# heathsc/bs_call

Measured on AMD Instinct MI355X. Metric: genome positions called/sec, higher is better.
Workload: dtype f64

## Files before the change

### bs_call_amd/csrc/bscall_api.c

```c
#ifndef __HIP_PLATFORM_AMD__
#define __HIP_PLATFORM_AMD__ 1
#endif
#include <hip/hip_runtime_api.h>
#include <math.h>
#include <pthread.h>
#include <stdarg.h>
#include <stdio.h>
#include <stdlib.h>
#include <string.h>

#include "../../include/bscall_amd.h"
#include "devtables.h"
#include "bsmath.h"
#include "bsmath_tables.h"
#include "synth.h"
#include "dbsnpdev_core.h"

int bsc_dev_launch_call(const void *cts, const void *ref, uint64_t n, void *out, uint32_t out_dw, void *skip,
                        const void *tb, void *het_list, void *counters, int num_cus, void *stream, void *ev_start,
                        void *ev_mid, void *ev_stop);
int bsc_dev_launch_accumulate(const void *rd, const void *bin_off, const void *seq, uint32_t x, uint32_t y, uint32_t min_qual, void *cts,
                              void *counters, int num_cus, void *stream);
int bsc_dev_launch_bin_reads(const void *tpl, uint32_t nr, const void *seq, uint64_t seq_bytes, uint32_t x, uint32_t y, void *tflag,
                             void *bin_cnt, void *bin_off, void *bin_cur, void *scan_tmp, size_t scan_tmp_bytes, void *rd,
// ... 25 lines not shown
size_t bsc_dev_chain_het_bytes(uint32_t n, int num_cus, int with_depth, int reads);
size_t bsc_dev_chain_scratch_bytes(int num_cus);
size_t bsc_dev_chain_multi_table_bytes(uint32_t n_blocks);
int bsc_dev_launch_chain_multi(const bsc_chain_launch *L, const bsc_chain_mblock *blk, uint32_t b_first, uint32_t b_last, void *tab_h,
                               void *tab_d, size_t *cursor);
int bsc_dev_launch_accumulate_summary(const void *rd, const void *bin_off, const void *seq, uint32_t x, uint32_t y, uint32_t min_qual, void *cts,
                                      void *counters, int num_cus, void *stream);
size_t bsc_dev_summary_bytes(void);
int bsc_dev_launch_accumulate_multi(const void *rd, const void *bin_off, const void *seq, const void *d_blk, uint32_t n_blk, uint32_t n_bins,
                                    uint32_t min_qual, void *cts, void *counters, int num_cus, void *stream);
int bsc_dev_scan_tmp_bytes_u64(uint32_t n, size_t *bytes);
size_t bsc_dev_prep_plan_bytes(void);
int bsc_dev_launch_prep(const void *raw, uint32_t nr, const void *seq, uint64_t seq_bytes, const void *misms, uint64_t n_misms,
                        const bsc_prep_params *par, void *ms_work, void *plan, void *out_len, void *out_off, void *scan_tmp,
                        size_t scan_tmp_bytes, void *tpl_out, void *seq_out, uint64_t seq_out_cap, void *cnt, int num_cus, void *stream,
                        const void *prof_ref, uint32_t prof_x, uint32_t prof_n_ref, uint32_t prof_cap, uint32_t prof_used0, void *prof_table,
                        void *max_pos1, void *used_scan, void *prof_mask);
int bsc_dev_launch_bcf(const void *recs, const void *core, const void *aux, const void *n_recs, uint64_t max_recs, int32_t rid,
                       const bsc_bcf_ids *ids, const void *name_pos, const void *name_off, const void *name_bytes, uint32_t n_names,
                       void *tile_bytes, void *tile_off, void *scan_tmp, size_t scan_tmp_bytes, void *out, uint64_t out_cap, void *totals,
                       int num_cus, void *stream, const void *emit_len);
int bsc_dev_launch_vcf_text(const void *recs, const void *core, const void *aux, const void *n_recs, uint64_t max_recs, const char *contig,
                            uint32_t contig_len, const void *name_pos, const void *name_off, const void *name_bytes, uint32_t n_names,
                            void *tile_bytes, void *tile_off, void *line_len, void *scan_tmp, size_t scan_tmp_bytes, void *out, uint64_t out_cap,
                            void *totals, int num_cus, void *stream);
int bsc_dev_launch_fmt_g(const void *v, uint64_t n, void *out16, int num_cus, void *stream);
int bsc_dev_launch_meth(const void *recs, const void *core, const void *aux, const void *n_recs, uint64_t max_recs, const void *emit, const char *contig,
                        uint32_t contig_len, const bsc_meth_params *par, void *tile_bytes, void *tile_off, void *line_len, void *scan_tmp,
                        size_t scan_tmp_bytes, void *out, uint64_t out_cap, void *totals, int num_cus, void *stream);
int bsc_dev_launch_ref_pad(const void *packed, const void *d_blk, uint32_t n_blk, void *padded, uint32_t n_pos, int num_cus, void *stream);
int bsc_dev_launch_bin_reads_multi(const void *tpl, uint32_t nr, const void *seq, uint64_t seq_bytes, const void *d_blk, uint32_t n_blk,
                                   uint32_t n_bins, void *tflag, void *bin_cnt, void *bin_off, void *bin_cur, void *scan_tmp,
// ... 131 lines not shown
  size_t cap_pmask;
  void *d_pprof, *d_pmax, *d_pused;
  size_t cap_pprof, cap_pmax, cap_pused;
  void *d_refp;
  size_t cap_refp;
  const uint32_t *mb_toff;
  int dbg_fail_summary;
  int reads_fused;
  void *d_fscr;
  size_t cap_fscr;
  hipEvent_t ev_rchain[2];
  int ev_rchain_valid;
  hipEvent_t ev_raw[2];
  int ev_raw_valid;
  int ref_resident;
  hipEvent_t ev_acc[2];
  int ev_acc_valid;
  hipStream_t s_in, s_out;
  hipEvent_t ev_in[2], ev_k[2], ev_out[2];
  void *p_cts[2], *p_ref[2], *p_out[2], *p_skip[2];
  size_t p_cap_cts[2], p_cap_ref[2], p_cap_out[2], p_cap_skip[2];
  int pipe_ready;
  int profiling;
#define BSC_EV_RING 32
  hipEvent_t ev[BSC_EV_RING][3];
  uint64_t ev_count;
};

static __thread char bsc_errbuf[512];

// ... 153 lines not shown
  HIP_TRY(hipGetDeviceProperties(&prop, dev));
  if (strncmp(prop.gcnArchName, "gfx950", 6) != 0)
    return bsc_fail(BSC_ERR_NO_DEVICE, "bsc_create: device %d is %s; the kernels are built for gfx950 only", dev,
                    prop.gcnArchName);

  bsc_context *ctx = calloc(1, sizeof *ctx);
  if (!ctx) return bsc_fail(BSC_ERR_NOMEM, "bsc_create: out of host memory");
  ctx->params = p;
  ctx->device = dev;
  ctx->num_cus = prop.multiProcessorCount;
  ctx->max_launch = BSC_MAX_LAUNCH;
  ctx->rec_share = 0.55;
  ctx->stage_timing = getenv("BSC_STAGE_TIMING") != NULL;
  ctx->no_emit_bytes = getenv("BSC_NO_EMIT_BYTES") != NULL;
  ctx->no_h2d_turns = getenv("BSC_NO_H2D_TURNS") != NULL;
  {
    const char *ml = getenv("BSC_MAX_LAUNCH_SITES");
    if (ml && *ml) {
      const unsigned long long v = strtoull(ml, NULL, 10) & ~63ull;
      if (v >= 64 && v < BSC_MAX_LAUNCH) ctx->max_launch = v;
    }
  }
  bsc_build_tables(ctx);
  int rc = BSC_OK;
  if (bsc_build_phred_table(&ctx->host_tables)) {
    rc = bsc_fail(BSC_ERR_ARG, "bsc_create: the QUAL staircase of this build's log is not monotone");
    bsc_destroy(ctx);
    return rc;
  }
  if (hipStreamCreateWithFlags(&ctx->stream, hipStreamNonBlocking) != hipSuccess ||
// ... 50 lines not shown
  hipFree(ctx->d_bcnt);
  hipFree(ctx->d_boff);
  hipFree(ctx->d_bcur);
  hipFree(ctx->d_bscan);
  for (int b = 0; b < 2; b++) {
    hipFree(ctx->p_cts[b]);
    hipFree(ctx->p_ref[b]);
    hipFree(ctx->p_out[b]);
    hipFree(ctx->p_skip[b]);
    if (ctx->ev_in[b]) hipEventDestroy(ctx->ev_in[b]);
    if (ctx->ev_k[b]) hipEventDestroy(ctx->ev_k[b]);
    if (ctx->ev_out[b]) hipEventDestroy(ctx->ev_out[b]);
  }
  if (ctx->s_in) hipStreamDestroy(ctx->s_in);
  if (ctx->s_out) hipStreamDestroy(ctx->s_out);
  hipFree(ctx->d_vg);
  hipFree(ctx->d_sstats);
    hipFree(ctx->d_pairs);
  hipFree(ctx->d_tcnt);
  hipFree(ctx->d_toff);
  hipFree(ctx->d_scantmp);
  hipFree(ctx->d_recs);
  hipFree(ctx->d_btb);
  hipFree(ctx->d_bto);
  hipFree(ctx->d_bscn);
  hipFree(ctx->d_bnm);
  hipFree(ctx->dbs.d_blob);
  bsc_dev_dbsnp_flat_free(&ctx->dbs.blob);
  if (ctx->h_names) hipHostFree(ctx->h_names);
  for (int k = 0; k < 4; k++)
// ... 121 lines not shown
                                ctx->profiling ? ctx->ev[ctx->ev_count % BSC_EV_RING][0] : NULL,
                                ctx->profiling ? ctx->ev[ctx->ev_count % BSC_EV_RING][1] : NULL,
                                ctx->profiling ? ctx->ev[ctx->ev_count % BSC_EV_RING][2] : NULL);
    if (ctx->profiling) ctx->ev_count++;
    if (e) return bsc_fail(BSC_ERR_HIP, "kernel launch failed: %s", hipGetErrorString((hipError_t)e));
    done += m;
  }
  ctx->sites += n;
  return BSC_OK;
}

#define BSC_PIPE_CHUNK (1u << 20)

static int bsc_pipe_init(bsc_context *ctx) {
  if (ctx->pipe_ready) return BSC_OK;
  HIP_TRY(hipStreamCreateWithFlags(&ctx->s_in, hipStreamNonBlocking));
  HIP_TRY(hipStreamCreateWithFlags(&ctx->s_out, hipStreamNonBlocking));
  for (int b = 0; b < 2; b++) {
    HIP_TRY(hipEventCreateWithFlags(&ctx->ev_in[b], hipEventDisableTiming));
    HIP_TRY(hipEventCreateWithFlags(&ctx->ev_k[b], hipEventDisableTiming));
    HIP_TRY(hipEventCreateWithFlags(&ctx->ev_out[b], hipEventDisableTiming));
  }
  ctx->pipe_ready = 1;
  return BSC_OK;
}

int bsc_call_sites(bsc_context *ctx, const bsc_pileup *cts, const uint8_t *ref, uint64_t n, void *out,
                   uint32_t out_stride, uint8_t *skip) {
  if (!ctx) return bsc_fail(BSC_ERR_ARG, "bsc_call_sites: ctx is NULL");
  int rc = bsc_check_stride(out_stride);
  if (rc) return rc;
// ... 688 lines not shown
  L.cts = d_cts;
  if (ctx->profiling) {
    if (!ctx->ev_chain[0])
      for (int i = 0; i < 2; i++) HIP_TRY(hipEventCreate(&ctx->ev_chain[i]));
    L.ev_start = ctx->ev_chain[0];
    L.ev_stop = ctx->ev_chain[1];
    ctx->ev_chain_valid = 1;
  }
  int e = bsc_dev_launch_chain(&L);
  if (e) return bsc_fail(BSC_ERR_HIP, "chain launch failed: %s", hipGetErrorString((hipError_t)e));
  if (with_stats) ctx->carry_slot ^= 1u;
  ctx->sites += w->n;
  return BSC_OK;
}

static int bsc_reads_chain_queue(bsc_context *ctx, const void *d_tpl, uint32_t nr, const void *d_seq, uint64_t seq_bytes, uint32_t x,
                                 uint32_t y, const void *d_ref, const void *d_dbsnp, const bsc_vcf_params *params, int with_stats,
                                 void *d_core, void *d_aux, void *d_emit, hipStream_t s) {
  const uint64_t sz64 = (uint64_t)y - x + 1;
  bsc_window w = {x, (uint32_t)sz64, 0u, (uint32_t)sz64};
  int rc = bsc_window_check("reads chain", &w);
  if (rc) return rc;
  size_t scan_bytes = 0;
  if ((rc = bsc_accumulate_reserve(ctx, nr, x, y, &scan_bytes))) return rc;
  if ((rc = bsc_reserve(&ctx->d_fscr, &ctx->cap_fscr, bsc_dev_chain_scratch_bytes(ctx->num_cus)))) return rc;
  bsc_chain_launch L;
  if ((rc = bsc_chain_fill(ctx, &L, &w, params, with_stats, 1, d_ref, d_dbsnp, d_core, d_aux, s))) return rc;
  L.emit_out = d_emit;
  if (ctx->profiling) {
    if (!ctx->ev_rchain[0])
// ... 6 lines not shown
  if (two_kernels) {
    const size_t n_pad = ((size_t)w.n + 63u) / 64u * 64u;
    size_t need = n_pad * bsc_dev_summary_bytes();
    if (ctx->dbg_fail_summary) {
      void *never = NULL;
      size_t cap0 = 0;
      if (!bsc_try_reserve(&never, &cap0, (size_t)1 << 60)) need = 0;
      else hipFree(never);
    }
    if (!need || !bsc_try_reserve(&ctx->d_cts, &ctx->cap_cts, need)) two_kernels = 0;
  }
  if (two_kernels) {
    e = bsc_dev_launch_accumulate_summary(ctx->d_rd, ctx->d_boff, d_seq, x, y, (uint32_t)ctx->params.min_qual, ctx->d_cts,
                                          ctx->d_counters, ctx->num_cus, s);
    if (e) return bsc_fail(BSC_ERR_HIP, "accumulate launch failed: %s", hipGetErrorString((hipError_t)e));
    bsc_chain_launch L2 = L;
    L.cts = ctx->d_cts;
    L.cts_summary = 1;
    L.run_if = 2;
    e = bsc_dev_launch_chain(&L);
    if (e) return bsc_fail(BSC_ERR_HIP, "reads chain launch failed: %s", hipGetErrorString((hipError_t)e));
    L = L2;
    L.run_if = 1;
    L.ev_start = NULL;
  }
  if (!two_kernels || L.run_if) {
    L.rd = ctx->d_rd;
    L.bin_off = ctx->d_boff;
    L.seq = d_seq;
    L.f_scratch = ctx->d_fscr;
    L.n_bins = bsc_dev_n_bins(w.n);
    L.min_qual = (uint32_t)ctx->params.min_qual;
  }
  e = bsc_dev_launch_chain(&L);
  if (e) return bsc_fail(BSC_ERR_HIP, "reads chain launch failed: %s", hipGetErrorString((hipError_t)e));
  if (ctx->profiling) {
    HIP_TRY(hipEventRecord(ctx->ev_rchain[1], s));
    ctx->ev_rchain_valid = 1;
  }
  if (with_stats) ctx->carry_slot ^= 1u;
  ctx->sites += w.n;
  return BSC_OK;
}

int bsc_reads_chain_device(bsc_context *ctx, const void *d_tpl, uint32_t nr, const void *d_seq, uint64_t seq_bytes, uint32_t x,
                           uint32_t y, const void *d_ref, const void *d_dbsnp, const bsc_vcf_params *params, int with_stats,
                           void *d_core, void *d_aux, void *stream) {
  if (!ctx || !params || !d_ref || !d_core) return bsc_fail(BSC_ERR_ARG, "bsc_reads_chain_device: NULL argument");
// ... 107 lines not shown
  free(so);
  if (rc >= 0 || strstr(bsc_errbuf, "seq_out too small"))
    return bsc_fail(BSC_ERR_ARG, "bsc_prepare_templates_device: template %u fails check %u on the device, none on the host", ti, code);
  char msg[sizeof bsc_errbuf];
  snprintf(msg, sizeof msg, "%s", bsc_errbuf);
  char *at = strstr(msg, "template 0 ");
  if (at) {
    char tail[sizeof bsc_errbuf];
    snprintf(tail, sizeof tail, "%s", at + 11);
    *at = 0;
    return bsc_fail(rc, "%stemplate %u %s", msg, ti, tail);
  }
  return bsc_fail(rc, "%s (template %u)", msg, ti);
}

static int bsc_prep_queue(bsc_context *ctx, const void *d_raw, uint32_t nr, const void *d_seq, uint64_t seq_bytes, const void *d_misms, uint64_t n_misms,
                          const bsc_prep_params *par, void *d_tpl_out, void *d_seq_out, uint64_t seq_out_cap, const bsc_read_profile *pf, hipStream_t s) {
  int rc;
  size_t scan_bytes = 0;
  const uint32_t n2 = 2u * nr + 1u;
  if (bsc_dev_scan_tmp_bytes_u64(n2, &scan_bytes)) return bsc_fail(BSC_ERR_HIP, "bsc_prepare_templates_device: scan size query failed");
  if ((rc = bsc_reserve(&ctx->d_pplan, &ctx->cap_pplan, (size_t)(nr ? nr : 1) * 2u * bsc_dev_prep_plan_bytes()))) return rc;
  if ((rc = bsc_reserve(&ctx->d_plen, &ctx->cap_plen, (size_t)n2 * 8u))) return rc;
  if ((rc = bsc_reserve(&ctx->d_poff, &ctx->cap_poff, (size_t)n2 * 8u))) return rc;
  if ((rc = bsc_reserve(&ctx->d_pms, &ctx->cap_pms, (size_t)(n_misms ? n_misms : 1) * sizeof(bsc_misms)))) return rc;
  if ((rc = bsc_reserve(&ctx->d_pscan, &ctx->cap_pscan, scan_bytes ? scan_bytes : 1))) return rc;
  if ((rc = bsc_reserve(&ctx->d_pcnt, &ctx->cap_pcnt, BSC_PREP_CNT_ALL * sizeof(unsigned long long)))) return rc;
  const size_t prof_bytes = pf && nr ? (size_t)pf->cap * 4u * sizeof(unsigned long long) : 0;
  const size_t h_need = (BSC_PREP_CNT_ALL + 2u) * sizeof(unsigned long long) + prof_bytes;
  if (h_need > ctx->cap_hprep) {
    if (ctx->h_prep) hipHostFree(ctx->h_prep);
    ctx->h_prep = NULL;
    ctx->cap_hprep = 0;
    if (hipHostMalloc((void **)&ctx->h_prep, h_need, hipHostMallocDefault) != hipSuccess)
      return bsc_fail(BSC_ERR_NOMEM, "bsc_prepare_templates_device: hipHostMalloc(%zu) failed", h_need);
    ctx->cap_hprep = h_need;
  }
  if (prof_bytes) {
    if ((rc = bsc_reserve(&ctx->d_pprof, &ctx->cap_pprof, prof_bytes))) return rc;
    if ((rc = bsc_reserve(&ctx->d_pmax, &ctx->cap_pmax, (size_t)nr * 4u))) return rc;
    if ((rc = bsc_reserve(&ctx->d_pused, &ctx->cap_pused, (size_t)nr * 4u))) return rc;
    if ((rc = bsc_reserve(&ctx->d_pmask, &ctx->cap_pmask, (size_t)pf->n_ref + 28u))) return rc;
    HIP_TRY(hipMemsetAsync(ctx->d_pprof, 0, prof_bytes, s));
  }
  HIP_TRY(hipMemsetAsync(ctx->d_pcnt, 0, BSC_PREP_CNT_ALL * sizeof(unsigned long long), s));
  HIP_TRY(hipMemsetAsync(ctx->d_pcnt, 0xff, sizeof(unsigned long long), s));
  int e = bsc_dev_launch_prep(d_raw, nr, d_seq, seq_bytes, d_misms, n_misms, par, ctx->d_pms, ctx->d_pplan, ctx->d_plen, ctx->d_poff,
                              ctx->d_pscan, scan_bytes, d_tpl_out, d_seq_out, seq_out_cap, ctx->d_pcnt, ctx->num_cus, s,
                              prof_bytes ? pf->ref : NULL, pf ? pf->x : 0u, pf ? pf->n_ref : 0u, pf ? pf->cap : 0u, pf ? pf->used : 0u,
                              ctx->d_pprof, ctx->d_pmax, ctx->d_pused, ctx->d_pmask);
  if (e) {
    (void)hipStreamSynchronize(s);
    return bsc_fail(BSC_ERR_HIP, "read pre-processing launch failed: %s", hipGetErrorString((hipError_t)e));
  }
  unsigned long long *h = ctx->h_prep;
  h[BSC_PREP_CNT_ALL + 1u] = 0;
  HIP_TRY(hipMemcpyAsync(h, ctx->d_pcnt, BSC_PREP_CNT_ALL * sizeof(unsigned long long), hipMemcpyDeviceToHost, s));
  HIP_TRY(hipMemcpyAsync(h + BSC_PREP_CNT_ALL, (const char *)ctx->d_poff + (size_t)(nr ? 2u * nr : 0u) * 8u, sizeof(unsigned long long), hipMemcpyDeviceToHost, s));
  if (prof_bytes) {
    HIP_TRY(hipMemcpyAsync(h + BSC_PREP_CNT_ALL + 2u, ctx->d_pprof, prof_bytes, hipMemcpyDeviceToHost, s));
    HIP_TRY(hipMemcpyAsync(h + BSC_PREP_CNT_ALL + 1u, (const char *)ctx->d_pused + (size_t)(nr - 1u) * 4u, 4, hipMemcpyDeviceToHost, s));
  }
  return BSC_OK;
}

static int bsc_prep_finish(bsc_context *ctx, const void *d_raw, uint32_t nr, const void *d_seq, const void *d_misms, const bsc_prep_params *par,
                           uint64_t *seq_out_used, bsc_prep_stats *stats, bsc_read_profile *pf) {
  const unsigned long long *hs = ctx->h_prep;
  unsigned long long h[8];
  memcpy(h, hs, sizeof h);
  for (unsigned k = 0; k < BSC_PREP_CNT_SLOTS; k++) {
    h[1] += hs[8u + 8u * k];
    h[2] += hs[8u + 8u * k + 1u];
  }
  if (h[0] != ~0ull) return bsc_prep_device_error(ctx, h[0], d_raw, d_seq, d_misms, par);
  if (pf && nr) {
    const uint32_t used_last = (uint32_t)hs[BSC_PREP_CNT_ALL + 1u];
    const unsigned long long *delta = hs + BSC_PREP_CNT_ALL + 2u;
// ... 430 lines not shown
  pthread_mutex_unlock(&bsc_h2d_lock);
}

static void bsc_h2d_turn_forget(bsc_context *ctx) {
  pthread_mutex_lock(&bsc_h2d_lock);
  if (bsc_h2d_last_ctx == ctx) {
    bsc_h2d_last = NULL;
    bsc_h2d_last_ctx = NULL;
    bsc_h2d_last_dev = -1;
  }
  pthread_mutex_unlock(&bsc_h2d_lock);
  if (ctx->ev_h2d) (void)hipEventDestroy(ctx->ev_h2d);
  ctx->ev_h2d = NULL;
}

static int bsc_records_queue(bsc_context *ctx, const bsc_template *tpl, uint32_t nr, const uint8_t *seq, uint64_t seq_bytes, uint32_t x,
                             uint32_t y, const uint8_t *ref, const uint8_t *dbsnp, const bsc_vcf_params *params, int with_stats,
                             bsc_vcf_rec *out, uint64_t out_cap, int stage, const bsc_bcf_req *bcf) {
  const int resident = stage == 2;
  if (resident) {
    stage = 0;
    tpl = NULL;
  }
  if (y < x) return bsc_fail(BSC_ERR_ARG, "accumulate: y (%u) < x (%u) (reference asserts y >= x)", y, x);
  if (nr && !resident && (!tpl || !seq)) return bsc_fail(BSC_ERR_ARG, "accumulate: NULL template or read buffer");
  if (ctx->pending_sz || ctx->rec_pending)
    return bsc_fail(BSC_ERR_ARG, "a submitted block has not been fetched (bsc_block_fetch / bsc_block_records_fetch first)");
  const uint64_t sz64 = (uint64_t)y - x + 1;
  if (sz64 > 0x0fffffffull) return bsc_fail(BSC_ERR_ARG, "bsc_block_records: block longer than 2^28 - 1 positions");
  const uint32_t sz = (uint32_t)sz64;
// ... 37 lines not shown
      memcpy(st + o_db, dbsnp, b_db);
      dbsnp = (const uint8_t *)(st + o_db);
    }
  }
  hipStream_t s = ctx->stream;
  ctx->blk_tpl = tpl;
  ctx->blk_d_tpl = ctx->d_tpl;
  ctx->blk_x = x;
  ctx->mb_n = 0;
  const int turns = bcf != NULL && !resident;
  if (turns) bsc_h2d_turn_begin(ctx, s);
  if (nr && !resident) {
    HIP_TRY(hipMemcpyAsync(ctx->d_tpl, tpl, (size_t)nr * sizeof(bsc_template), hipMemcpyHostToDevice, s));
    HIP_TRY(hipMemcpyAsync(ctx->d_seq, seq, (size_t)seq_bytes, hipMemcpyHostToDevice, s));
  }
  if (!(resident && ctx->ref_resident)) HIP_TRY(hipMemcpyAsync(ctx->d_ref, ref, (size_t)sz + 2, hipMemcpyHostToDevice, s));
  if (dbsnp) HIP_TRY(hipMemcpyAsync(ctx->d_vdb, dbsnp, (size_t)sz, hipMemcpyHostToDevice, s));
  if (bcf && (rc = bsc_names_upload(ctx, "bsc_block_bcf", bcf->names, s))) return rc;
  if (att_names && (rc = bsc_names_attached(ctx, x, sz, s))) return rc;
  const bsc_bcf_names *const names_ready = ctx->names_up;
  const bsc_bcf_names *const enc_names = att_names ? names_ready : (bcf ? bcf->names : NULL);
  ctx->names_up = NULL;
  if (turns) bsc_h2d_turn_end(ctx, s);
  if (att_flags) {
    const int e = bsc_dev_launch_dbsnp_flags(&ctx->dbs.dev, x, sz, ctx->d_vdb, ctx->num_cus, s);
    if (e) return bsc_fail(BSC_ERR_HIP, "dbSNP flags launch failed: %s", hipGetErrorString((hipError_t)e));
  }
  void *d_db = dbsnp || att_flags ? ctx->d_vdb : NULL;
  void *d_emit = NULL;
  if (!ctx->no_emit_bytes) {
    if ((rc = bsc_reserve(&ctx->d_emit, &ctx->cap_emit, (size_t)sz + 64u))) return rc;
// ... 188 lines not shown
  clock_gettime(CLOCK_MONOTONIC, &t);
  return (double)t.tv_sec + 1e-9 * (double)t.tv_nsec;
}
static int bsc_block_records_rawdev_(bsc_context *ctx, const void *d_raw, uint32_t nr, const void *d_rseq, uint64_t seq_bytes, const void *d_rms,
                                     uint64_t n_misms, uint64_t cap, const bsc_prep_params *prep, uint32_t x, uint32_t y, const uint8_t *ref,
                                     const uint8_t *dbsnp, const bsc_vcf_params *params, int with_stats, bsc_vcf_rec *out, uint64_t out_cap,
                                     uint64_t *n_out, bsc_prep_stats *prep_stats, bsc_read_profile *profile, const bsc_bcf_req *bcf) {
  int rc;
  const int timing = ctx->stage_timing;
  double t0 = timing ? bsc_now_s() : 0.0, t1;
  if ((rc = bsc_reserve(&ctx->d_tpl, &ctx->cap_tpl, (size_t)nr * sizeof(bsc_template)))) return rc;
  if ((rc = bsc_reserve(&ctx->d_seq, &ctx->cap_seq, (size_t)cap))) return rc;
  hipStream_t s = ctx->stream;
  bsc_read_profile dp;
  ctx->ref_resident = 0;
  if (profile) {
    const uint64_t n_ref = (uint64_t)y - x + 3;
    if ((rc = bsc_reserve(&ctx->d_ref, &ctx->cap_ref, (size_t)n_ref))) return rc;
    HIP_TRY(hipMemcpyAsync(ctx->d_ref, ref, (size_t)n_ref, hipMemcpyHostToDevice, s));
    ctx->ref_resident = 1;
    dp = *profile;
    dp.ref = ctx->d_ref;
    dp.x = x;
    dp.n_ref = (uint32_t)n_ref;
  }
  if (ctx->profiling) {
    if (!ctx->ev_raw[0])
      for (int i = 0; i < 2; i++) HIP_TRY(hipEventCreate(&ctx->ev_raw[i]));
    HIP_TRY(hipEventRecord(ctx->ev_raw[0], s));
    ctx->ev_raw_valid = 0;
  }
  if (timing) {
    t1 = bsc_now_s();
    fprintf(stderr, "bsc stage: reserve + reference upload queued %.1f us\n", (t1 - t0) * 1e6);
    t0 = t1;
  }
  if ((rc = bsc_prep_args_check(ctx, d_raw, nr, d_rseq, seq_bytes, d_rms, n_misms, prep, ctx->d_tpl, ctx->d_seq, cap, profile ? &dp : NULL))) return rc;
  if (prep_stats) memset(prep_stats, 0, sizeof *prep_stats);
  if ((rc = bsc_prep_queue(ctx, d_raw, nr, d_rseq, seq_bytes, d_rms, n_misms, prep, ctx->d_tpl, ctx->d_seq, cap, profile ? &dp : NULL, s))) {
    (void)hipStreamSynchronize(s);
    return rc;
  }
  if (timing) {
    t1 = bsc_now_s();
    fprintf(stderr, "bsc stage: pre-processing queued %.1f us\n", (t1 - t0) * 1e6);
    t0 = t1;
  }
  rc = bsc_records_queue(ctx, NULL, nr, NULL, cap, x, y, ref, dbsnp, params, with_stats, out, out_cap, 2, bcf);
  ctx->ref_resident = 0;
  if (rc) {
    (void)hipStreamSynchronize(ctx->stream);
    return rc;
  }
  if (ctx->profiling && hipEventRecord(ctx->ev_raw[1], s) == hipSuccess) ctx->ev_raw_valid = 1;
  if (timing) {
    t1 = bsc_now_s();
    fprintf(stderr, "bsc stage: bsc_records_queue (reserves, uploads, launches) %.1f us\n", (t1 - t0) * 1e6);
    t0 = t1;
  }
  const hipError_t se = hipStreamSynchronize(s);
  if (se != hipSuccess) return bsc_fail(BSC_ERR_HIP, "bsc_block_records_raw: %s", hipGetErrorString(se));
  if (timing) {
    t1 = bsc_now_s();
    fprintf(stderr, "bsc stage: the wait %.1f us\n", (t1 - t0) * 1e6);
    t0 = t1;
  }
  rc = bsc_prep_finish(ctx, d_raw, nr, d_rseq, d_rms, prep, NULL, prep_stats, profile ? &dp : NULL);
  if (profile) profile->used = dp.used;
  if (rc) {
    ctx->bcf_out = NULL;
    ctx->bcf_blk = 0;
    return rc;
  }
  rc = bsc_records_finish(ctx, n_out);
  if (timing) {
    t1 = bsc_now_s();
    fprintf(stderr, "bsc stage: bsc_records_finish %.1f us\n", (t1 - t0) * 1e6);
  }
  return rc;
}

static int bsc_block_records_raw_(bsc_context *ctx, const bsc_raw_template *raw, uint32_t nr, const uint8_t *seq, uint64_t seq_bytes,
                                  const bsc_misms *misms, uint64_t n_misms, const bsc_prep_params *prep, uint32_t x, uint32_t y, const uint8_t *ref,
                                  const uint8_t *dbsnp, const bsc_vcf_params *params, int with_stats, bsc_vcf_rec *out, uint64_t out_cap,
                                  uint64_t *n_out, bsc_prep_stats *prep_stats, bsc_read_profile *profile, const bsc_bcf_req *bcf) {
  if (!ctx || !ref || !params || !prep || !n_out || (!out && out_cap)) return bsc_fail(BSC_ERR_ARG, "bsc_block_records_raw: NULL argument");
  if (y < x) return bsc_fail(BSC_ERR_ARG, "bsc_block_records_raw: y (%u) < x (%u)", y, x);
  *n_out = 0;
  if (prep_stats) memset(prep_stats, 0, sizeof *prep_stats);
  if (ctx->rec_pending || ctx->pending_sz) return bsc_fail(BSC_ERR_ARG, "bsc_block_records_raw: a submitted block has not been fetched");
  if (nr && (!raw || (seq_bytes && !seq) || (n_misms && !misms))) return bsc_fail(BSC_ERR_ARG, "bsc_block_records_raw: NULL input buffer");
  if (!nr) return bsc_block_records_(ctx, NULL, 0, NULL, 0, x, y, ref, dbsnp, params, with_stats, out, out_cap, n_out, bcf);
  if (y - x > 0x0ffffffeu) return bsc_fail(BSC_ERR_ARG, "bsc_block_records_raw: block longer than 2^28 - 1 positions");
// ... 1553 lines not shown
```

### bs_call_amd/csrc/prepdev.hip

```cpp
#include <hip/hip_runtime.h>
#include <stdint.h>

#include "../../include/bscall_amd.h"

#define FLT_QUAL 63u

struct bsc_prep_plan {
  uint64_t src;
  uint64_t ms;
  uint32_t rl0;
  uint32_t w0, wl;
  uint32_t nm;
  uint32_t mark_l, mark_r;
  uint32_t out_len;
  uint32_t present;
  uint32_t trim_l, trim_r;
};

struct bsc_prep_desc {
  uint64_t srcw;
  uint32_t pk;
  int32_t pc;
};
#define PD_PRESENT 1u
// ... 815 lines not shown
  flush();
  __syncthreads();
  for (unsigned i = threadIdx.x; i < PROF_LDS * 4u; i += 64 * PREP_WAVES)
    if (s_prof[i] && i % PROF_LDS < F.cap) atomicAdd(&F.table[(uint64_t)(i % PROF_LDS) * 4u + i / PROF_LDS], (unsigned long long)s_prof[i]);
}

extern "C" int bsc_dev_scan_u64(const void *in, void *out, uint32_t n, void *tmp, size_t tmp_bytes, void *stream);

extern "C" size_t bsc_dev_prep_plan_bytes(void) { return sizeof(bsc_prep_plan) + sizeof(bsc_prep_desc); }

extern "C" int bsc_dev_scan_max_u32(const void *in, void *out, uint32_t n, void *tmp, size_t tmp_bytes, void *stream);

extern "C" int bsc_dev_launch_prep(const void *raw, uint32_t nr, const void *seq, uint64_t seq_bytes, const void *misms, uint64_t n_misms,
                                   const bsc_prep_params *par, void *ms_work, void *plan, void *out_len, void *out_off, void *scan_tmp,
                                   size_t scan_tmp_bytes, void *tpl_out, void *seq_out, uint64_t seq_out_cap, void *cnt, int num_cus,
                                   void *stream, const void *prof_ref, uint32_t prof_x, uint32_t prof_n_ref, uint32_t prof_cap,
                                   uint32_t prof_used0, void *prof_table, void *max_pos1, void *used_scan, void *prof_mask) {
  hipStream_t s = (hipStream_t)stream;
  bsc_prep_desc *const desc = (bsc_prep_desc *)((bsc_prep_plan *)plan + 2ull * nr);
  if (!nr) return (int)hipMemsetAsync(out_off, 0, sizeof(unsigned long long), s);
  hipError_t e = hipMemsetAsync((unsigned long long *)out_len + 2ull * nr, 0, sizeof(unsigned long long), s);
  if (e != hipSuccess) return (int)e;
  hipLaunchKernelGGL(bsc_prep_plan_kernel, dim3((nr + 255u) / 256u), dim3(256), 0, s, (const bsc_raw_template *)raw, nr, (const uint8_t *)seq,
                     seq_bytes, (const bsc_misms *)misms, n_misms, *par, (bsc_misms *)ms_work, (bsc_prep_plan *)plan, desc,
                     (unsigned long long *)out_len, (bsc_template *)tpl_out, (unsigned long long *)cnt, prof_ref ? (uint32_t *)max_pos1 : nullptr);
  if ((e = hipGetLastError()) != hipSuccess) return (int)e;
  int rc = bsc_dev_scan_u64(out_len, out_off, 2u * nr + 1u, scan_tmp, scan_tmp_bytes, stream);
  if (rc) return rc;
  bsc_prep_prof F = {nullptr, 0u, 0u, 0u, 0u, nullptr, nullptr};
  if (prof_ref) {
    if ((rc = bsc_dev_scan_max_u32(max_pos1, used_scan, nr, scan_tmp, scan_tmp_bytes, stream))) return rc;
    F.ref = (const uint8_t *)prof_ref;
    F.x = prof_x;
    F.n_ref = prof_n_ref;
    F.cap = prof_cap;
    F.used0 = prof_used0;
    F.used_scan = (const uint32_t *)used_scan;
    F.table = (unsigned long long *)prof_table;
  }
  unsigned g = ((nr + 31u) / 32u + PREP_WAVES - 1u) / PREP_WAVES;
  static int per_cu[2] = {0, 0};
  for (int pv = 0; pv < (prof_ref ? 2 : 1); pv++)
    if (!per_cu[pv]) {
      int nb = 0;
      const hipError_t eo = pv ? hipOccupancyMaxActiveBlocksPerMultiprocessor(&nb, bsc_prep_profile_kernel, 64 * PREP_WAVES, 0)
                               : hipOccupancyMaxActiveBlocksPerMultiprocessor(&nb, bsc_prep_copy_kernel, 64 * PREP_WAVES, 0);
      per_cu[pv] = (eo == hipSuccess && nb > 0) ? nb : 4;
      (void)hipGetLastError();
    }
  unsigned gc = g, gp = g;
  if (gc > (unsigned)num_cus * (unsigned)per_cu[0]) gc = (unsigned)num_cus * (unsigned)per_cu[0];
  hipLaunchKernelGGL(bsc_prep_copy_kernel, dim3(gc), dim3(64 * PREP_WAVES), 0, s, (const bsc_prep_plan *)plan, (const bsc_prep_desc *)desc, nr,
                     (const uint8_t *)seq, (const bsc_misms *)ms_work, (const unsigned long long *)out_off, par->min_qual, (bsc_template *)tpl_out,
                     (uint8_t *)seq_out, seq_out_cap, (unsigned long long *)cnt);
  if ((e = hipGetLastError()) != hipSuccess) return (int)e;
  if (prof_ref) {
    hipLaunchKernelGGL(bsc_prep_refmask_kernel, dim3((unsigned)(((uint64_t)prof_n_ref + 24u + 1023u) / 1024u)), dim3(256), 0, s, (const uint8_t *)prof_ref,
                       prof_n_ref, (uint8_t *)prof_mask);
    if ((e = hipGetLastError()) != hipSuccess) return (int)e;
    if (gp > (unsigned)num_cus * (unsigned)per_cu[1]) gp = (unsigned)num_cus * (unsigned)per_cu[1];
    hipLaunchKernelGGL(bsc_prep_profile_kernel, dim3(gp), dim3(64 * PREP_WAVES), 0, s, (const bsc_prep_plan *)plan, (const bsc_prep_desc *)desc, nr,
                       (const bsc_misms *)ms_work, (const unsigned long long *)out_off, (const bsc_template *)tpl_out, (const uint8_t *)seq_out,
                       seq_out_cap, (unsigned long long *)cnt, (const uint8_t *)prof_mask, F);
  }
  return (int)hipGetLastError();
}
```

Measured before the change: 18.00 billion.

## Overlap reference upload and read-profile kernels with main pipeline on side streams

Splits read pre-processing into front, profile and back stages. The reference upload moves to a separate input stream, and the profile kernels (refmask plus profile) run on a low-priority side stream, both joined back with events. The main-stream chain launch waits on the reference-ready event only just before it needs the reference. The aim is to hide the H2D copy and the profiling kernels behind prep and accumulate work, at the cost of more events, streams and cross-stream synchronisation.

```diff
diff --git a/bs_call_amd/csrc/bscall_api.c b/bs_call_amd/csrc/bscall_api.c
--- a/bs_call_amd/csrc/bscall_api.c
+++ b/bs_call_amd/csrc/bscall_api.c
@@ -63,8 +63,11 @@
 int bsc_dev_launch_prep(const void *raw, uint32_t nr, const void *seq, uint64_t seq_bytes, const void *misms, uint64_t n_misms,
                         const bsc_prep_params *par, void *ms_work, void *plan, void *out_len, void *out_off, void *scan_tmp,
                         size_t scan_tmp_bytes, void *tpl_out, void *seq_out, uint64_t seq_out_cap, void *cnt, int num_cus, void *stream,
-                        const void *prof_ref, uint32_t prof_x, uint32_t prof_n_ref, uint32_t prof_cap, uint32_t prof_used0, void *prof_table,
-                        void *max_pos1, void *used_scan, void *prof_mask);
+                        int prof, void *max_pos1, void *used_scan);
+int bsc_dev_launch_prep_profile(uint32_t nr, const void *ms_work, const void *plan, const void *out_off, const void *tpl_out, const void *seq_out,
+                                uint64_t seq_out_cap, void *cnt, int num_cus, void *stream, const void *prof_ref, uint32_t prof_x,
+                                uint32_t prof_n_ref, uint32_t prof_cap, uint32_t prof_used0, void *prof_table, const void *used_scan,
+                                void *prof_mask);
 int bsc_dev_launch_bcf(const void *recs, const void *core, const void *aux, const void *n_recs, uint64_t max_recs, int32_t rid,
                        const bsc_bcf_ids *ids, const void *name_pos, const void *name_off, const void *name_bytes, uint32_t n_names,
                        void *tile_bytes, void *tile_off, void *scan_tmp, size_t scan_tmp_bytes, void *out, uint64_t out_cap, void *totals,
@@ -226,6 +229,11 @@
   hipEvent_t ev_raw[2];
   int ev_raw_valid;
   int ref_resident;
+  int raw_serial;
+  hipStream_t s_side;
+  hipEvent_t ev_head, ev_up, ev_fork, ev_join;
+  int ref_async;
+  hipEvent_t ref_ready;
   hipEvent_t ev_acc[2];
   int ev_acc_valid;
   hipStream_t s_in, s_out;
@@ -409,6 +417,7 @@
   ctx->stage_timing = getenv("BSC_STAGE_TIMING") != NULL;
   ctx->no_emit_bytes = getenv("BSC_NO_EMIT_BYTES") != NULL;
   ctx->no_h2d_turns = getenv("BSC_NO_H2D_TURNS") != NULL;
+  ctx->raw_serial = getenv("BSC_RAW_SERIAL") != NULL;
   {
     const char *ml = getenv("BSC_MAX_LAUNCH_SITES");
     if (ml && *ml) {
@@ -489,6 +498,11 @@
   }
   if (ctx->s_in) hipStreamDestroy(ctx->s_in);
   if (ctx->s_out) hipStreamDestroy(ctx->s_out);
+  if (ctx->s_side) hipStreamDestroy(ctx->s_side);
+  if (ctx->ev_head) hipEventDestroy(ctx->ev_head);
+  if (ctx->ev_up) hipEventDestroy(ctx->ev_up);
+  if (ctx->ev_fork) hipEventDestroy(ctx->ev_fork);
+  if (ctx->ev_join) hipEventDestroy(ctx->ev_join);
   hipFree(ctx->d_vg);
   hipFree(ctx->d_sstats);
     hipFree(ctx->d_pairs);
@@ -640,7 +654,7 @@
 
 static int bsc_pipe_init(bsc_context *ctx) {
   if (ctx->pipe_ready) return BSC_OK;
-  HIP_TRY(hipStreamCreateWithFlags(&ctx->s_in, hipStreamNonBlocking));
+  if (!ctx->s_in) HIP_TRY(hipStreamCreateWithFlags(&ctx->s_in, hipStreamNonBlocking));
   HIP_TRY(hipStreamCreateWithFlags(&ctx->s_out, hipStreamNonBlocking));
   for (int b = 0; b < 2; b++) {
     HIP_TRY(hipEventCreateWithFlags(&ctx->ev_in[b], hipEventDisableTiming));
@@ -1359,6 +1373,14 @@
   return BSC_OK;
 }
 
+static int bsc_ref_ready_wait(bsc_context *ctx, hipStream_t s) {
+  if (!ctx->ref_ready) return BSC_OK;
+  const hipEvent_t ev = ctx->ref_ready;
+  ctx->ref_ready = NULL;
+  HIP_TRY(hipStreamWaitEvent(s, ev, 0));
+  return BSC_OK;
+}
+
 static int bsc_reads_chain_queue(bsc_context *ctx, const void *d_tpl, uint32_t nr, const void *d_seq, uint64_t seq_bytes, uint32_t x,
                                  uint32_t y, const void *d_ref, const void *d_dbsnp, const bsc_vcf_params *params, int with_stats,
                                  void *d_core, void *d_aux, void *d_emit, hipStream_t s) {
@@ -1395,6 +1417,7 @@
     e = bsc_dev_launch_accumulate_summary(ctx->d_rd, ctx->d_boff, d_seq, x, y, (uint32_t)ctx->params.min_qual, ctx->d_cts,
                                           ctx->d_counters, ctx->num_cus, s);
     if (e) return bsc_fail(BSC_ERR_HIP, "accumulate launch failed: %s", hipGetErrorString((hipError_t)e));
+    if ((rc = bsc_ref_ready_wait(ctx, s))) return rc;
     bsc_chain_launch L2 = L;
     L.cts = ctx->d_cts;
     L.cts_summary = 1;
@@ -1413,6 +1436,7 @@
     L.n_bins = bsc_dev_n_bins(w.n);
     L.min_qual = (uint32_t)ctx->params.min_qual;
   }
+  if ((rc = bsc_ref_ready_wait(ctx, s))) return rc;
   e = bsc_dev_launch_chain(&L);
   if (e) return bsc_fail(BSC_ERR_HIP, "reads chain launch failed: %s", hipGetErrorString((hipError_t)e));
   if (ctx->profiling) {
@@ -1550,8 +1574,10 @@
   return bsc_fail(rc, "%s (template %u)", msg, ti);
 }
 
-static int bsc_prep_queue(bsc_context *ctx, const void *d_raw, uint32_t nr, const void *d_seq, uint64_t seq_bytes, const void *d_misms, uint64_t n_misms,
-                          const bsc_prep_params *par, void *d_tpl_out, void *d_seq_out, uint64_t seq_out_cap, const bsc_read_profile *pf, hipStream_t s) {
+static size_t bsc_prep_prof_bytes(const bsc_read_profile *pf, uint32_t nr) { return pf && nr ? (size_t)pf->cap * 4u * sizeof(unsigned long long) : 0; }
+
+static int bsc_prep_queue_front(bsc_context *ctx, const void *d_raw, uint32_t nr, const void *d_seq, uint64_t seq_bytes, const void *d_misms, uint64_t n_misms,
+                                const bsc_prep_params *par, void *d_tpl_out, void *d_seq_out, uint64_t seq_out_cap, const bsc_read_profile *pf, hipStream_t s) {
   int rc;
   size_t scan_bytes = 0;
   const uint32_t n2 = 2u * nr + 1u;
@@ -1562,7 +1588,7 @@
   if ((rc = bsc_reserve(&ctx->d_pms, &ctx->cap_pms, (size_t)(n_misms ? n_misms : 1) * sizeof(bsc_misms)))) return rc;
   if ((rc = bsc_reserve(&ctx->d_pscan, &ctx->cap_pscan, scan_bytes ? scan_bytes : 1))) return rc;
   if ((rc = bsc_reserve(&ctx->d_pcnt, &ctx->cap_pcnt, BSC_PREP_CNT_ALL * sizeof(unsigned long long)))) return rc;
-  const size_t prof_bytes = pf && nr ? (size_t)pf->cap * 4u * sizeof(unsigned long long) : 0;
+  const size_t prof_bytes = bsc_prep_prof_bytes(pf, nr);
   const size_t h_need = (BSC_PREP_CNT_ALL + 2u) * sizeof(unsigned long long) + prof_bytes;
   if (h_need > ctx->cap_hprep) {
     if (ctx->h_prep) hipHostFree(ctx->h_prep);
@@ -1582,13 +1608,26 @@
   HIP_TRY(hipMemsetAsync(ctx->d_pcnt, 0, BSC_PREP_CNT_ALL * sizeof(unsigned long long), s));
   HIP_TRY(hipMemsetAsync(ctx->d_pcnt, 0xff, sizeof(unsigned long long), s));
   int e = bsc_dev_launch_prep(d_raw, nr, d_seq, seq_bytes, d_misms, n_misms, par, ctx->d_pms, ctx->d_pplan, ctx->d_plen, ctx->d_poff,
-                              ctx->d_pscan, scan_bytes, d_tpl_out, d_seq_out, seq_out_cap, ctx->d_pcnt, ctx->num_cus, s,
-                              prof_bytes ? pf->ref : NULL, pf ? pf->x : 0u, pf ? pf->n_ref : 0u, pf ? pf->cap : 0u, pf ? pf->used : 0u,
-                              ctx->d_pprof, ctx->d_pmax, ctx->d_pused, ctx->d_pmask);
+                              ctx->d_pscan, scan_bytes, d_tpl_out, d_seq_out, seq_out_cap, ctx->d_pcnt, ctx->num_cus, s, prof_bytes != 0,
+                              ctx->d_pmax, ctx->d_pused);
   if (e) {
     (void)hipStreamSynchronize(s);
     return bsc_fail(BSC_ERR_HIP, "read pre-processing launch failed: %s", hipGetErrorString((hipError_t)e));
   }
+  return BSC_OK;
+}
+
+static int bsc_prep_queue_profile(bsc_context *ctx, uint32_t nr, void *d_tpl_out, void *d_seq_out, uint64_t seq_out_cap, const bsc_read_profile *pf,
+                                  hipStream_t s) {
+  if (!bsc_prep_prof_bytes(pf, nr)) return BSC_OK;
+  int e = bsc_dev_launch_prep_profile(nr, ctx->d_pms, ctx->d_pplan, ctx->d_poff, d_tpl_out, d_seq_out, seq_out_cap, ctx->d_pcnt, ctx->num_cus, s,
+                                      pf->ref, pf->x, pf->n_ref, pf->cap, pf->used, ctx->d_pprof, ctx->d_pused, ctx->d_pmask);
+  if (e) return bsc_fail(BSC_ERR_HIP, "read pre-processing launch failed: %s", hipGetErrorString((hipError_t)e));
+  return BSC_OK;
+}
+
+static int bsc_prep_queue_back(bsc_context *ctx, uint32_t nr, const bsc_read_profile *pf, hipStream_t s) {
+  const size_t prof_bytes = bsc_prep_prof_bytes(pf, nr);
   unsigned long long *h = ctx->h_prep;
   h[BSC_PREP_CNT_ALL + 1u] = 0;
   HIP_TRY(hipMemcpyAsync(h, ctx->d_pcnt, BSC_PREP_CNT_ALL * sizeof(unsigned long long), hipMemcpyDeviceToHost, s));
@@ -1598,6 +1637,17 @@
     HIP_TRY(hipMemcpyAsync(h + BSC_PREP_CNT_ALL + 1u, (const char *)ctx->d_pused + (size_t)(nr - 1u) * 4u, 4, hipMemcpyDeviceToHost, s));
   }
   return BSC_OK;
+}
+
+static int bsc_prep_queue(bsc_context *ctx, const void *d_raw, uint32_t nr, const void *d_seq, uint64_t seq_bytes, const void *d_misms, uint64_t n_misms,
+                          const bsc_prep_params *par, void *d_tpl_out, void *d_seq_out, uint64_t seq_out_cap, const bsc_read_profile *pf, hipStream_t s) {
+  int rc = bsc_prep_queue_front(ctx, d_raw, nr, d_seq, seq_bytes, d_misms, n_misms, par, d_tpl_out, d_seq_out, seq_out_cap, pf, s);
+  if (rc) return rc;
+  if ((rc = bsc_prep_queue_profile(ctx, nr, d_tpl_out, d_seq_out, seq_out_cap, pf, s))) {
+    (void)hipStreamSynchronize(s);
+    return rc;
+  }
+  return bsc_prep_queue_back(ctx, nr, pf, s);
 }
 
 static int bsc_prep_finish(bsc_context *ctx, const void *d_raw, uint32_t nr, const void *d_seq, const void *d_misms, const bsc_prep_params *par,
@@ -2058,6 +2108,40 @@
   ctx->ev_h2d = NULL;
 }
 
+static int bsc_raw_streams(bsc_context *ctx) {
+  if (ctx->raw_serial) return 0;
+  if (ctx->s_side) return 1;
+  int least = 0, greatest = 0;
+  if (hipDeviceGetStreamPriorityRange(&least, &greatest) != hipSuccess) least = greatest = 0;
+  hipError_t e = ctx->s_in ? hipSuccess : hipStreamCreateWithFlags(&ctx->s_in, hipStreamNonBlocking);
+  hipEvent_t *const evs[4] = {&ctx->ev_head, &ctx->ev_up, &ctx->ev_fork, &ctx->ev_join};
+  for (int i = 0; i < 4 && e == hipSuccess; i++)
+    if (!*evs[i]) e = hipEventCreateWithFlags(evs[i], hipEventDisableTiming);
+  if (e == hipSuccess)
+    e = least != greatest ? hipStreamCreateWithPriority(&ctx->s_side, hipStreamNonBlocking, least) : hipStreamCreateWithFlags(&ctx->s_side, hipStreamNonBlocking);
+  if (e != hipSuccess) {
+    (void)hipGetLastError();
+    ctx->s_side = NULL;
+    ctx->raw_serial = 1;
+    return 0;
+  }
+  return 1;
+}
+
+static int bsc_raw_ref_upload(bsc_context *ctx, const uint8_t *ref, size_t bytes) {
+  HIP_TRY(hipStreamWaitEvent(ctx->s_in, ctx->ev_head, 0));
+  HIP_TRY(hipMemcpyAsync(ctx->d_ref, ref, bytes, hipMemcpyHostToDevice, ctx->s_in));
+  HIP_TRY(hipEventRecord(ctx->ev_up, ctx->s_in));
+  ctx->ref_ready = ctx->ev_up;
+  return BSC_OK;
+}
+
+static void bsc_raw_quiesce(bsc_context *ctx) {
+  (void)hipStreamSynchronize(ctx->stream);
+  if (ctx->s_in) (void)hipStreamSynchronize(ctx->s_in);
+  if (ctx->s_side) (void)hipStreamSynchronize(ctx->s_side);
+}
+
 static int bsc_records_queue(bsc_context *ctx, const bsc_template *tpl, uint32_t nr, const uint8_t *seq, uint64_t seq_bytes, uint32_t x,
                              uint32_t y, const uint8_t *ref, const uint8_t *dbsnp, const bsc_vcf_params *params, int with_stats,
                              bsc_vcf_rec *out, uint64_t out_cap, int stage, const bsc_bcf_req *bcf) {
@@ -2125,7 +2209,10 @@
     HIP_TRY(hipMemcpyAsync(ctx->d_tpl, tpl, (size_t)nr * sizeof(bsc_template), hipMemcpyHostToDevice, s));
     HIP_TRY(hipMemcpyAsync(ctx->d_seq, seq, (size_t)seq_bytes, hipMemcpyHostToDevice, s));
   }
-  if (!(resident && ctx->ref_resident)) HIP_TRY(hipMemcpyAsync(ctx->d_ref, ref, (size_t)sz + 2, hipMemcpyHostToDevice, s));
+  if (resident && ctx->ref_async) {
+    if (!ctx->ref_resident && (rc = bsc_raw_ref_upload(ctx, ref, (size_t)sz + 2))) return rc;
+  } else if (!(resident && ctx->ref_resident))
+    HIP_TRY(hipMemcpyAsync(ctx->d_ref, ref, (size_t)sz + 2, hipMemcpyHostToDevice, s));
   if (dbsnp) HIP_TRY(hipMemcpyAsync(ctx->d_vdb, dbsnp, (size_t)sz, hipMemcpyHostToDevice, s));
   if (bcf && (rc = bsc_names_upload(ctx, "bsc_block_bcf", bcf->names, s))) return rc;
   if (att_names && (rc = bsc_names_attached(ctx, x, sz, s))) return rc;
@@ -2344,11 +2431,12 @@
   hipStream_t s = ctx->stream;
   bsc_read_profile dp;
   ctx->ref_resident = 0;
+  ctx->ref_ready = NULL;
+  const int overlap = bsc_raw_streams(ctx);
+  const uint64_t n_ref = (uint64_t)y - x + 3;
   if (profile) {
-    const uint64_t n_ref = (uint64_t)y - x + 3;
     if ((rc = bsc_reserve(&ctx->d_ref, &ctx->cap_ref, (size_t)n_ref))) return rc;
-    HIP_TRY(hipMemcpyAsync(ctx->d_ref, ref, (size_t)n_ref, hipMemcpyHostToDevice, s));
-    ctx->ref_resident = 1;
+    if (!overlap) HIP_TRY(hipMemcpyAsync(ctx->d_ref, ref, (size_t)n_ref, hipMemcpyHostToDevice, s));
     dp = *profile;
     dp.ref = ctx->d_ref;
     dp.x = x;
@@ -2360,27 +2448,48 @@
     HIP_TRY(hipEventRecord(ctx->ev_raw[0], s));
     ctx->ev_raw_valid = 0;
   }
+  if (overlap) HIP_TRY(hipEventRecord(ctx->ev_head, s));
   if (timing) {
     t1 = bsc_now_s();
     fprintf(stderr, "bsc stage: reserve + reference upload queued %.1f us\n", (t1 - t0) * 1e6);
     t0 = t1;
   }
-  if ((rc = bsc_prep_args_check(ctx, d_raw, nr, d_rseq, seq_bytes, d_rms, n_misms, prep, ctx->d_tpl, ctx->d_seq, cap, profile ? &dp : NULL))) return rc;
+  if ((rc = bsc_prep_args_check(ctx, d_raw, nr, d_rseq, seq_bytes, d_rms, n_misms, prep, ctx->d_tpl, ctx->d_seq, cap, profile ? &dp : NULL))) goto fail;
   if (prep_stats) memset(prep_stats, 0, sizeof *prep_stats);
-  if ((rc = bsc_prep_queue(ctx, d_raw, nr, d_rseq, seq_bytes, d_rms, n_misms, prep, ctx->d_tpl, ctx->d_seq, cap, profile ? &dp : NULL, s))) {
-    (void)hipStreamSynchronize(s);
-    return rc;
-  }
+  if ((rc = bsc_prep_queue_front(ctx, d_raw, nr, d_rseq, seq_bytes, d_rms, n_misms, prep, ctx->d_tpl, ctx->d_seq, cap, profile ? &dp : NULL, s))) goto fail;
+  int forked = 0;
+  if (profile) {
+    if (overlap && (rc = bsc_raw_ref_upload(ctx, ref, (size_t)n_ref))) goto fail;
+    ctx->ref_resident = 1;
+    hipStream_t sp = s;
+    if (overlap && nr) {
+      sp = ctx->s_side;
+      forked = 1;
+      if (hipEventRecord(ctx->ev_fork, s) != hipSuccess || hipStreamWaitEvent(sp, ctx->ev_fork, 0) != hipSuccess ||
+          hipStreamWaitEvent(sp, ctx->ev_up, 0) != hipSuccess) {
+        rc = bsc_fail(BSC_ERR_HIP, "bsc_block_records_raw: %s", hipGetErrorString(hipGetLastError()));
+        goto fail;
+      }
+    }
+    if ((rc = bsc_prep_queue_profile(ctx, nr, ctx->d_tpl, ctx->d_seq, cap, &dp, sp))) goto fail;
+  }
+  if (!forked && (rc = bsc_prep_queue_back(ctx, nr, profile ? &dp : NULL, s))) goto fail;
   if (timing) {
     t1 = bsc_now_s();
     fprintf(stderr, "bsc stage: pre-processing queued %.1f us\n", (t1 - t0) * 1e6);
     t0 = t1;
   }
+  ctx->ref_async = overlap;
   rc = bsc_records_queue(ctx, NULL, nr, NULL, cap, x, y, ref, dbsnp, params, with_stats, out, out_cap, 2, bcf);
-  ctx->ref_resident = 0;
-  if (rc) {
-    (void)hipStreamSynchronize(ctx->stream);
-    return rc;
+  ctx->ref_resident = ctx->ref_async = 0;
+  if (!rc) rc = bsc_ref_ready_wait(ctx, s);
+  if (rc) goto fail;
+  if (forked) {
+    if (hipEventRecord(ctx->ev_join, ctx->s_side) != hipSuccess || hipStreamWaitEvent(s, ctx->ev_join, 0) != hipSuccess) {
+      rc = bsc_fail(BSC_ERR_HIP, "bsc_block_records_raw: %s", hipGetErrorString(hipGetLastError()));
+      goto fail;
+    }
+    if ((rc = bsc_prep_queue_back(ctx, nr, &dp, s))) goto fail;
   }
   if (ctx->profiling && hipEventRecord(ctx->ev_raw[1], s) == hipSuccess) ctx->ev_raw_valid = 1;
   if (timing) {
@@ -2389,7 +2498,10 @@
     t0 = t1;
   }
   const hipError_t se = hipStreamSynchronize(s);
-  if (se != hipSuccess) return bsc_fail(BSC_ERR_HIP, "bsc_block_records_raw: %s", hipGetErrorString(se));
+  if (se != hipSuccess) {
+    bsc_raw_quiesce(ctx);
+    return bsc_fail(BSC_ERR_HIP, "bsc_block_records_raw: %s", hipGetErrorString(se));
+  }
   if (timing) {
     t1 = bsc_now_s();
     fprintf(stderr, "bsc stage: the wait %.1f us\n", (t1 - t0) * 1e6);
@@ -2407,6 +2519,11 @@
     t1 = bsc_now_s();
     fprintf(stderr, "bsc stage: bsc_records_finish %.1f us\n", (t1 - t0) * 1e6);
   }
+  return rc;
+fail:
+  ctx->ref_resident = ctx->ref_async = 0;
+  ctx->ref_ready = NULL;
+  bsc_raw_quiesce(ctx);
   return rc;
 }
 
diff --git a/bs_call_amd/csrc/prepdev.hip b/bs_call_amd/csrc/prepdev.hip
--- a/bs_call_amd/csrc/prepdev.hip
+++ b/bs_call_amd/csrc/prepdev.hip
@@ -853,8 +853,7 @@
 extern "C" int bsc_dev_launch_prep(const void *raw, uint32_t nr, const void *seq, uint64_t seq_bytes, const void *misms, uint64_t n_misms,
                                    const bsc_prep_params *par, void *ms_work, void *plan, void *out_len, void *out_off, void *scan_tmp,
                                    size_t scan_tmp_bytes, void *tpl_out, void *seq_out, uint64_t seq_out_cap, void *cnt, int num_cus,
-                                   void *stream, const void *prof_ref, uint32_t prof_x, uint32_t prof_n_ref, uint32_t prof_cap,
-                                   uint32_t prof_used0, void *prof_table, void *max_pos1, void *used_scan, void *prof_mask) {
+                                   void *stream, int prof, void *max_pos1, void *used_scan) {
   hipStream_t s = (hipStream_t)stream;
   bsc_prep_desc *const desc = (bsc_prep_desc *)((bsc_prep_plan *)plan + 2ull * nr);
   if (!nr) return (int)hipMemsetAsync(out_off, 0, sizeof(unsigned long long), s);
@@ -862,45 +861,49 @@
   if (e != hipSuccess) return (int)e;
   hipLaunchKernelGGL(bsc_prep_plan_kernel, dim3((nr + 255u) / 256u), dim3(256), 0, s, (const bsc_raw_template *)raw, nr, (const uint8_t *)seq,
                      seq_bytes, (const bsc_misms *)misms, n_misms, *par, (bsc_misms *)ms_work, (bsc_prep_plan *)plan, desc,
-                     (unsigned long long *)out_len, (bsc_template *)tpl_out, (unsigned long long *)cnt, prof_ref ? (uint32_t *)max_pos1 : nullptr);
+                     (unsigned long long *)out_len, (bsc_template *)tpl_out, (unsigned long long *)cnt, prof ? (uint32_t *)max_pos1 : nullptr);
   if ((e = hipGetLastError()) != hipSuccess) return (int)e;
   int rc = bsc_dev_scan_u64(out_len, out_off, 2u * nr + 1u, scan_tmp, scan_tmp_bytes, stream);
   if (rc) return rc;
-  bsc_prep_prof F = {nullptr, 0u, 0u, 0u, 0u, nullptr, nullptr};
-  if (prof_ref) {
-    if ((rc = bsc_dev_scan_max_u32(max_pos1, used_scan, nr, scan_tmp, scan_tmp_bytes, stream))) return rc;
-    F.ref = (const uint8_t *)prof_ref;
-    F.x = prof_x;
-    F.n_ref = prof_n_ref;
-    F.cap = prof_cap;
-    F.used0 = prof_used0;
-    F.used_scan = (const uint32_t *)used_scan;
-    F.table = (unsigned long long *)prof_table;
-  }
+  if (prof && (rc = bsc_dev_scan_max_u32(max_pos1, used_scan, nr, scan_tmp, scan_tmp_bytes, stream))) return rc;
   unsigned g = ((nr + 31u) / 32u + PREP_WAVES - 1u) / PREP_WAVES;
-  static int per_cu[2] = {0, 0};
-  for (int pv = 0; pv < (prof_ref ? 2 : 1); pv++)
-    if (!per_cu[pv]) {
-      int nb = 0;
-      const hipError_t eo = pv ? hipOccupancyMaxActiveBlocksPerMultiprocessor(&nb, bsc_prep_profile_kernel, 64 * PREP_WAVES, 0)
-                               : hipOccupancyMaxActiveBlocksPerMultiprocessor(&nb, bsc_prep_copy_kernel, 64 * PREP_WAVES, 0);
-      per_cu[pv] = (eo == hipSuccess && nb > 0) ? nb : 4;
-      (void)hipGetLastError();
-    }
-  unsigned gc = g, gp = g;
-  if (gc > (unsigned)num_cus * (unsigned)per_cu[0]) gc = (unsigned)num_cus * (unsigned)per_cu[0];
-  hipLaunchKernelGGL(bsc_prep_copy_kernel, dim3(gc), dim3(64 * PREP_WAVES), 0, s, (const bsc_prep_plan *)plan, (const bsc_prep_desc *)desc, nr,
+  static int per_cu = 0;
+  if (!per_cu) {
+    int nb = 0;
+    const hipError_t eo = hipOccupancyMaxActiveBlocksPerMultiprocessor(&nb, bsc_prep_copy_kernel, 64 * PREP_WAVES, 0);
+    per_cu = (eo == hipSuccess && nb > 0) ? nb : 4;
+    (void)hipGetLastError();
+  }
+  if (g > (unsigned)num_cus * (unsigned)per_cu) g = (unsigned)num_cus * (unsigned)per_cu;
+  hipLaunchKernelGGL(bsc_prep_copy_kernel, dim3(g), dim3(64 * PREP_WAVES), 0, s, (const bsc_prep_plan *)plan, (const bsc_prep_desc *)desc, nr,
                      (const uint8_t *)seq, (const bsc_misms *)ms_work, (const unsigned long long *)out_off, par->min_qual, (bsc_template *)tpl_out,
                      (uint8_t *)seq_out, seq_out_cap, (unsigned long long *)cnt);
-  if ((e = hipGetLastError()) != hipSuccess) return (int)e;
-  if (prof_ref) {
-    hipLaunchKernelGGL(bsc_prep_refmask_kernel, dim3((unsigned)(((uint64_t)prof_n_ref + 24u + 1023u) / 1024u)), dim3(256), 0, s, (const uint8_t *)prof_ref,
-                       prof_n_ref, (uint8_t *)prof_mask);
-    if ((e = hipGetLastError()) != hipSuccess) return (int)e;
-    if (gp > (unsigned)num_cus * (unsigned)per_cu[1]) gp = (unsigned)num_cus * (unsigned)per_cu[1];
-    hipLaunchKernelGGL(bsc_prep_profile_kernel, dim3(gp), dim3(64 * PREP_WAVES), 0, s, (const bsc_prep_plan *)plan, (const bsc_prep_desc *)desc, nr,
-                       (const bsc_misms *)ms_work, (const unsigned long long *)out_off, (const bsc_template *)tpl_out, (const uint8_t *)seq_out,
-                       seq_out_cap, (unsigned long long *)cnt, (const uint8_t *)prof_mask, F);
-  }
   return (int)hipGetLastError();
 }
+
+extern "C" int bsc_dev_launch_prep_profile(uint32_t nr, const void *ms_work, const void *plan, const void *out_off, const void *tpl_out,
+                                           const void *seq_out, uint64_t seq_out_cap, void *cnt, int num_cus, void *stream, const void *prof_ref,
+                                           uint32_t prof_x, uint32_t prof_n_ref, uint32_t prof_cap, uint32_t prof_used0, void *prof_table,
+                                           const void *used_scan, void *prof_mask) {
+  hipStream_t s = (hipStream_t)stream;
+  if (!nr) return 0;
+  const bsc_prep_desc *const desc = (const bsc_prep_desc *)((const bsc_prep_plan *)plan + 2ull * nr);
+  const bsc_prep_prof F = {(const uint8_t *)prof_ref, prof_x, prof_n_ref, prof_cap, prof_used0, (const uint32_t *)used_scan, (unsigned long long *)prof_table};
+  hipLaunchKernelGGL(bsc_prep_refmask_kernel, dim3((unsigned)(((uint64_t)prof_n_ref + 24u + 1023u) / 1024u)), dim3(256), 0, s, (const uint8_t *)prof_ref,
+                     prof_n_ref, (uint8_t *)prof_mask);
+  hipError_t e = hipGetLastError();
+  if (e != hipSuccess) return (int)e;
+  static int per_cu = 0;
+  if (!per_cu) {
+    int nb = 0;
+    const hipError_t eo = hipOccupancyMaxActiveBlocksPerMultiprocessor(&nb, bsc_prep_profile_kernel, 64 * PREP_WAVES, 0);
+    per_cu = (eo == hipSuccess && nb > 0) ? nb : 4;
+    (void)hipGetLastError();
+  }
+  unsigned g = ((nr + 31u) / 32u + PREP_WAVES - 1u) / PREP_WAVES;
+  if (g > (unsigned)num_cus * (unsigned)per_cu) g = (unsigned)num_cus * (unsigned)per_cu;
+  hipLaunchKernelGGL(bsc_prep_profile_kernel, dim3(g), dim3(64 * PREP_WAVES), 0, s, (const bsc_prep_plan *)plan, desc, nr, (const bsc_misms *)ms_work,
+                     (const unsigned long long *)out_off, (const bsc_template *)tpl_out, (const uint8_t *)seq_out, seq_out_cap,
+                     (unsigned long long *)cnt, (const uint8_t *)prof_mask, F);
+  return (int)hipGetLastError();
+}
```

New measurement: 17.82 billion. 0.99x the previous value.
